# usra-riacs/Nonlocal-Monte-Carlo

Hardware: AMD Instinct MI355X
Metric: spin-updates/s (replicas x spins x sweeps / s), NPT sweep + swap rounds, schedule construction included (higher is better)
Workload: dtype f64 field + 53-bit uniform (the reference's arithmetic, NMC/nmc.py:86-87; on this +-J instance the fp64 field is an exact integer and the fp64 acceptance test an exact integer threshold per field value: bit-identical to the sweep-by-sweep fp64 kernel and the fp64 oracle); 1 GPU; NPT heat-bath sweeps + replica exchange, sparse +-J spin glass (C4 per GPU); spins=10000, edges=30000, replicas_per_gpu=256, replicas_total=256, sweeps_per_round=10, swap_pairs_per_round=77, rng=philox4x32-10, order=one permutation per sweep, plan_chunk_rounds=256

## Files before the change

### nonlocal-monte-carlo_amd/csrc/nlmc.hip

```cpp
#include "../../include/nlmc.h"
#include "nlmc_kernels.h"
#include "nlmc_pt_icm.h"
#include "nlmc_apt.h"
#include "nlmc_lbp.h"
#include "nlmc_nmc.h"
#include "nlmc_probe.h"
#include "nlmc_big.h"
#include "nlmc_host.h"

#include <dlfcn.h>

#include <algorithm>
#include <chrono>
#include <thread>
#include <climits>
#include <cmath>
#include <cstdio>
#include <cstdlib>
#include <cstring>
#include <string>
#include <vector>

namespace {

// ... 443 lines not shown
{
    const int waves = nt / 64;
    if (const char *s = getenv("NLMC_FUSED_GEN0")) { const int v = atoi(s); if (v >= 0 && v < waves) return v; }
    return waves / 2;
}

bool fused_supported(const nlmc_ctx *c, int T)
{
    if (getenv("NLMC_NO_FUSED") || c->big) return false;
    if (c->n < 256 || c->n > NLMC_FZ_SPT * 1024 || c->max_deg > 0x3FFF || T < 3 || T > NLMC_FUSED_TMAX) return false;
    if ((size_t)T * ((size_t)c->n + c->n_long) > ((size_t)1 << 22)) return false;
    if (c->n_pad + 16 > 0x3FFF) return false;
    (void)T;
    const FusedLds L = fused_lds(c->n, c->n_pad, true, false, false);
    if (3 * L.u_bytes / 4 > 0xFFFF) return false;
    return L.total <= (size_t)150 * 1024;
}

bool fused_f64_supported(const nlmc_ctx *c, int T)
{
    if (!c->f64_exact || c->xmax > 4095 || getenv("NLMC_NO_FUSED64")) return false;
    if (!fused_supported(c, T)) return false;
    return fused_lds(c->n, c->n_pad, false, false, fused_addr_format(c), 2 * c->xmax + 1).total <= (size_t)156 * 1024;
}

bool fused_f64_real_supported(const nlmc_ctx *c, int T)
{
    if (!c->f64_real || c->f64_exact || getenv("NLMC_NO_FUSED64")) return false;
    return fused_supported(c, T);
}

bool fused_f64_any(const nlmc_ctx *c, int T) { return fused_f64_supported(c, T) || fused_f64_real_supported(c, T); }

const void *fused_kernel(bool diag, bool flags, bool outs, int fmt, bool f64 = false, bool real = false)
{
    if (f64 && real) {
#define NLMC_KR(D, O) {reinterpret_cast<const void *>(k_sweep_fused<D, false, O, NLMC_FMT_WIDE, true, false, true>), \
                       reinterpret_cast<const void *>(k_sweep_fused<D, false, O, NLMC_FMT_COMPACT, true, false, true>), \
                       reinterpret_cast<const void *>(k_sweep_fused<D, false, O, NLMC_FMT_ADDR, true, false, true>)}
        static const void *const tr[2][2][3] = {{NLMC_KR(false, false), NLMC_KR(false, true)}, {NLMC_KR(true, false), NLMC_KR(true, true)}};
#undef NLMC_KR
        return flags ? nullptr : tr[diag][outs][fmt];
    }
    if (f64) {
#define NLMC_K64(D, O) {reinterpret_cast<const void *>(k_sweep_fused<D, false, O, NLMC_FMT_WIDE, true>), reinterpret_cast<const void *>(k_sweep_fused<D, false, O, NLMC_FMT_COMPACT, true>), \
                        reinterpret_cast<const void *>(k_sweep_fused<D, false, O, NLMC_FMT_ADDR, true>)}
        static const void *const t64[2][2][3] = {{NLMC_K64(false, false), NLMC_K64(false, true)}, {NLMC_K64(true, false), NLMC_K64(true, true)}};
#undef NLMC_K64
        return flags ? nullptr : t64[diag][outs][fmt];
    }
#define NLMC_K(D, F, O) {reinterpret_cast<const void *>(k_sweep_fused<D, F, O, NLMC_FMT_WIDE>), reinterpret_cast<const void *>(k_sweep_fused<D, F, O, NLMC_FMT_COMPACT>), \
                         reinterpret_cast<const void *>(k_sweep_fused<D, F, O, NLMC_FMT_ADDR>)}
    static const void *const table[2][2][2][3] = {{{NLMC_K(false, false, false), NLMC_K(false, false, true)}, {NLMC_K(false, true, false), NLMC_K(false, true, true)}},
                                                  {{NLMC_K(true, false, false), NLMC_K(true, false, true)}, {NLMC_K(true, true, false), NLMC_K(true, true, true)}}};
#undef NLMC_K
    static_assert(NLMC_FMT_WIDE == 0 && NLMC_FMT_COMPACT == 1 && NLMC_FMT_ADDR == 2, "table order");
    return table[diag][flags][outs][fmt];
}

struct SweepOut {
    int record_stride;
    int8_t *out_spins;
    double *out_energy;
    double *out_min_energy;
    int32_t *out_argmin;
    int8_t *out_argmin_state;
// ... 3 lines not shown
              bool outs, bool want_energy, bool want_min, bool want_state, int rec, int t0, int n_total, bool f64 = false,
              const DeferSwap *defer = nullptr, double *sink_override = nullptr)
{
    const nlmc_ctx::FusedPlan &P = c->fz[slot];
    const int R = c->sub_count(), n = c->n, T = P.T;
    const size_t PS = (size_t)P.pstride;
    const bool real = f64 && !c->f64_exact;
    if (real && !P.has_val) return fail(c, NLMC_ERR_STATE, "run_fused: the plan has no fp64 value plane");
    const int kt = (f64 && !real) ? 2 * c->xmax + 1 : 0;
    const bool snap_lds = outs && fused_lds(c->n, c->n_pad, c->has_flags, true, P.fmt == NLMC_FMT_ADDR, kt).total <= (size_t)150 * 1024;
    const FusedLds L = fused_lds(c->n, c->n_pad, c->has_flags, snap_lds, P.fmt == NLMC_FMT_ADDR, kt);
    if (outs && !snap_lds) HIP_TRY(c, c->snap_g.reserve((size_t)R * (3 * (size_t)c->n_pad + 16)));
    const int variant = (outs ? 4 : 0) + (c->has_diag ? 2 : 0) + (c->has_flags ? 1 : 0);
    const void *kfun = fused_kernel(c->has_diag, c->has_flags, outs, P.fmt, f64, real);
    int lds_slot = real ? 84 + ((c->has_diag ? 2 : 0) + (outs ? 1 : 0)) * 3 + P.fmt
                 : f64 ? 48 + ((c->has_diag ? 2 : 0) + (outs ? 1 : 0)) * 3 + P.fmt : 24 + variant * 3 + P.fmt;
    if (defer) {
#define NLMC_KD(D, F64_) {reinterpret_cast<const void *>(k_sweep_fused<D, false, false, NLMC_FMT_WIDE, F64_, true>), reinterpret_cast<const void *>(k_sweep_fused<D, false, false, NLMC_FMT_COMPACT, F64_, true>), \
                          reinterpret_cast<const void *>(k_sweep_fused<D, false, false, NLMC_FMT_ADDR, F64_, true>)}
        static const void *const dtable[2][2][3] = {{NLMC_KD(false, false), NLMC_KD(false, true)}, {NLMC_KD(true, false), NLMC_KD(true, true)}};
#undef NLMC_KD
        kfun = (c->has_flags || outs) ? nullptr : dtable[c->has_diag][f64][P.fmt];
        lds_slot = 72 + ((c->has_diag ? 2 : 0) + (f64 ? 1 : 0)) * 3 + P.fmt;
        if (real) {
#define NLMC_KDR(D) {reinterpret_cast<const void *>(k_sweep_fused<D, false, false, NLMC_FMT_WIDE, true, true, true>), \
                     reinterpret_cast<const void *>(k_sweep_fused<D, false, false, NLMC_FMT_COMPACT, true, true, true>), \
                     reinterpret_cast<const void *>(k_sweep_fused<D, false, false, NLMC_FMT_ADDR, true, true, true>)}
            static const void *const drtable[2][3] = {NLMC_KDR(false), NLMC_KDR(true)};
#undef NLMC_KDR
            kfun = (c->has_flags || outs) ? nullptr : drtable[c->has_diag][P.fmt];
            lds_slot = 96 + (c->has_diag ? 1 : 0) * 3 + P.fmt;
        }
    }
    if (!kfun) return fail(c, NLMC_ERR_STATE, "run_fused: no kernel for this combination (fp64 mode or deferred swap with phase flags / outputs)");
    { int rc = ensure_lds(c, lds_slot, kfun, L.total); if (rc) return rc; }
    const bool timed = c->ev_accumulate && (c->ev_every <= 1 || c->launches_total % c->ev_every == 0);
    hipEvent_t e0 = nullptr, e2 = nullptr;
    if (timed) {
        e0 = next_event(c);
        hipEvent_t e1 = next_event(c);
        e2 = next_event(c);
        if (!e0 || !e1 || !e2) return fail(c, NLMC_ERR_HIP, "hipEventCreate failed");
        tag_triple(c, 1);
        HIP_TRY(c, hipEventRecord(e0, c->cur));
    }
    SweepArgs a{};
    a.g = c->g;
    a.chain_base = c->chain_base;
    a.chain_list = c->sub_list();
    a.spins = c->spins.p;
    a.flags = c->has_flags ? c->flags.p : nullptr;
    a.temp_x = c->temp_x;
    a.lvl_off = P.loff.p + (size_t)w * (NLMC_LCAP + 1);
    a.nlev = P.nlev.p + w;
    a.hi_max = P.himax.p + w;
    a.ell32 = P.ell.p + (size_t)w * PS * NLMC_FZ_W;
    a.head32 = P.head.p + (size_t)w * PS;
    a.fsend = P.send.p + (size_t)w * T;
    a.fz_pstride = P.pstride;
    a.fz_fmt = P.fmt;
    if (w + 1 < P.windows && P.nlev_host[(size_t)w + 1] > 0 && !c->knob_no_warm) {
        a.warm_head = P.head.p + (size_t)(w + 1) * PS;
        a.warm_ell = P.ell.p + (size_t)(w + 1) * PS * NLMC_FZ_W;
        a.fz_npos_next = P.npos_host[(size_t)w + 1];
    }
    a.f_workers = P.workers;
    a.f_gen0 = P.gen0;
    a.f_gen_prio = c->knob_no_prio ? 0 : 1;
#ifdef NLMC_DEBUG_KNOBS
    a.dbg_flags = c->knob_dbg_flags;
#endif
    a.n_sweeps = T;
    a.sweep0 = sweep0;
    a.seed_lo = (uint32_t)seed; a.seed_hi = (uint32_t)(seed >> 32);
    a.tab = tab_dev; a.tab_cs = tab_cs; a.tab_ss = tab_ss;
    a.slot_of_chain = use_slots ? c->slot_of_chain.p : nullptr;
    a.efix = c->efix.p;
    a.energy_sink = sink_override ? sink_override : c->energy_sink;
    if (defer) a.defer = *defer;
    a.escale = c->escale;
    a.eshift = c->escale - c->qs;
    a.qinv = std::ldexp(1.0f, -c->qs);
    a.trace_sweeps = outs ? n_total : T;
    a.t0 = t0;
    a.rec_stride = rec ? rec : 1;
    a.min_stride = c->track_min ? c->track_min_stride : 1;
    a.argmin = c->argmin.p;
    if (outs) {
        a.etrace = want_energy ? c->etrace.p : nullptr;
        a.strace = rec ? c->strace.p : nullptr;
        a.emin = want_min ? c->emin.p : nullptr;
        a.best = (want_min && want_state) ? c->best.p : nullptr;
    }
    a.lds_neg_off = L.neg_off;
    a.lds_flags_off = L.flags_off; a.lds_u_off = L.u_off; a.lds_u_stride = L.u_bytes; a.lds_red_off = L.red_off;
    a.lds_snap_off = L.snap_off;
    a.snap_g = (outs && !snap_lds) ? c->snap_g.p : nullptr;
    a.lds_kt_off = L.kt_off;
    a.f64_xmax = c->xmax;
    a.f64_tie_mask = c->knob_tie_mask;
    a.qinv64 = std::ldexp(1.0, -c->qs);
    a.fz_val = real ? P.val.p + (size_t)w * NLMC_FZ_VAL_WORDS * PS : nullptr;
    a.rng_stride = c->rng_stride; a.rng_base = c->rng_base; a.rng_ladder_len = std::max(1, c->ladder_len);
#ifdef NLMC_STAMPS
    HIP_TRY(c, c->dbg.reserve((size_t)R * 16 * 8 + 96));
    HIP_TRY(c, hipMemsetAsync(c->dbg.p, 0, ((size_t)R * 16 * 8 + 96) * sizeof(long long), c->cur));
    a.dbg = c->dbg.p;
#endif
    const int nt = fused_block(n);
    void *kargs[] = {&a};
    HIP_TRY(c, hipLaunchKernel(kfun, dim3(R), dim3(nt), kargs, L.total, c->cur));
    HIP_TRY(c, hipGetLastError());
    if (timed) { HIP_TRY(c, hipEventRecord(e2, c->cur)); c->launches_timed++; }
    c->launches_sweep++;
    c->launches_total++;
    c->stat_fused_window = w;
    c->stat_fused_slot = slot;
    return NLMC_OK;
}

int read_sweep_outputs(nlmc_ctx *c, const SweepOut &o, int n_sweeps, int rec, int n_rec)
{
    const int R = c->sub_count(), RA = c->n_chains, n = c->n;
    bool need_sync = false;
    std::vector<long long> h_ll;
    if (o.out_energy) {
        h_ll.resize((size_t)R * n_sweeps);
        HIP_TRY(c, hipMemcpyAsync(h_ll.data(), c->etrace.p, sizeof(long long) * h_ll.size(), hipMemcpyDeviceToHost, c->cur));
// ... 2404 lines not shown
```

### nonlocal-monte-carlo_amd/csrc/nlmc_kernels.h

```cpp
#pragma once
#include "nlmc_device.h"

struct EdgeQ { int32_t col; int32_t q; };

struct CsrDev {
    int n, n_pad;
    const int32_t *rowptr;
    const int32_t *col;
    const double *val64;
    const EdgeQ *edge32;
    const double *h64;
    const int32_t *hq;
};

struct LevelizeArgs {
    CsrDev g;
    int n_orders;
    const uint32_t *keys_in;
    uint32_t seed_lo, seed_hi, sweep0;
    int per_chain;
    int n_sweeps;
    int chain_base;
    int level_cap;
    int two_sided;
// ... 1366 lines not shown
#endif
    chain_store(a, x);
}

template <int FMT> struct FusedItem {
    static constexpr int NE = NLMC_FZ_W;
    static constexpr int NP = FMT == NLMC_FMT_WIDE ? NE / 2 : FMT == NLMC_FMT_COMPACT ? NE / 4 : NE / 8;
    nlmc_i2 hd;
    nlmc_i4 pk[NP];
    __device__ __forceinline__ int word(int i) const { const int p = i >> 2, j = i & 3; return j == 0 ? pk[p].x : j == 1 ? pk[p].y : j == 2 ? pk[p].z : pk[p].w; }
    __device__ __forceinline__ unsigned col(int q) const
    {
        if (FMT == NLMC_FMT_WIDE) return (unsigned)word(2 * q);
        if (FMT == NLMC_FMT_COMPACT) return (unsigned)word(q) >> 16;
        return (q & 1) ? (unsigned)word(q >> 1) >> 16 : (unsigned)word(q >> 1) & 0xFFFFu;
    }
    __device__ __forceinline__ int val(int q) const
    {
        if (FMT == NLMC_FMT_WIDE) return word(2 * q + 1);
        return (int)(short)(word(q) & 0xFFFF);
    }
};

__device__ __forceinline__ float4 thresholds4(const u32x4 &r)
{
    float4 v;
    v.x = threshold_spec(r.x);
    v.y = threshold_spec(r.y);
    v.z = threshold_spec(r.z);
    v.w = threshold_spec(r.w);
    return v;
}

struct FusedGenParams { uint32_t gc; int gtid, gnt, nblk, nj, Tn; };
struct FusedWin {
    const int32_t *lvl_off;
    const int32_t *fsend;
    const EdgeQ *ell;
    const int2 *head;
    const int2 *warm_head;
    const EdgeQ *warm_ell;
    int npos_next;
    int nl, hi_max;
    uint32_t sweep0;
    const double *val;
};
struct FusedVals {
    nlmc_i4 v[NLMC_FZ_W / 2];
    nlmc_i2 h;
    __device__ __forceinline__ double val(int q) const
    {
        const nlmc_i4 &w = v[q >> 1];
        return (q & 1) ? __hiloint2double(w.w, w.z) : __hiloint2double(w.y, w.x);
    }
    __device__ __forceinline__ double field() const { return __hiloint2double(h.y, h.x); }
};
template <int CTRL>
__device__ __forceinline__ double quad_move_f64(double v)
{
    const long long b = __double_as_longlong(v);
    const int lo = __builtin_amdgcn_mov_dpp((int)b, CTRL, 0xF, 0xF, true), hi = __builtin_amdgcn_mov_dpp((int)(b >> 32), CTRL, 0xF, 0xF, true);
    return __hiloint2double(hi, lo);
}
#ifdef NLMC_DEBUG_KNOBS
#define NLMC_GEN_DBG_OFF_COND (a.dbg_flags & 1)
#define NLMC_GEN_DBG_PHILOX if (a.dbg_flags & 8) g_r = u32x4{(uint32_t)b * 2654435761u, (uint32_t)b ^ gp.gc, (uint32_t)g_u * 40503u + (uint32_t)b, ~(uint32_t)b}; else
#define NLMC_GEN_DBG_LOGIT if (a.dbg_flags & 16) dst[b] = nlmc_f4{__uint_as_float(g_r.x & 0x3FFFFFFFu), __uint_as_float(g_r.y & 0x3FFFFFFFu), __uint_as_float(g_r.z & 0x3FFFFFFFu), __uint_as_float(g_r.w & 0x3FFFFFFFu)}; else
#else
#define NLMC_GEN_DBG_OFF_COND false
#define NLMC_GEN_DBG_PHILOX
#define NLMC_GEN_DBG_LOGIT
#endif
#define NLMC_GEN_STATE int g_u = 2, g_slot = 2, g_w0 = 0, g_wend = 0, g_wlen = 1, g_acc = 0, g_sidx = 0; u32x4 g_r{0u, 0u, 0u, 0u}; \
    const uint32_t g_seed_lo = a.seed_lo, g_seed_hi = a.seed_hi, g_sweep0 = W.sweep0; const int g_u_off = a.lds_u_off, g_u_stride = a.lds_u_stride; \
    const int32_t *const g_fsend = W.fsend;
#define NLMC_GEN_NSTEP (g_f64 ? 2 : 3)
#define NLMC_GEN_ARM(a, gp)                                                                                             \
    {                                                                                                                   \
        typedef const int32_t __attribute__((address_space(4))) *const_i32_;                                            \
        g_sidx = 0; g_acc = 0;                                                                                          \
        if (g_u < gp.Tn) {                                                                                              \
            const const_i32_ send_ = (const_i32_)(uintptr_t)g_fsend;                                                    \
            g_w0 = g_u >= 3 ? __builtin_amdgcn_readfirstlane(send_[g_u - 3]) : -1;                                      \
            g_wend = __builtin_amdgcn_readfirstlane(send_[g_u - 2]);                                                    \
            g_wlen = max(1, g_wend - g_w0);                 \
        } else g_w0 = 0x7FFFFFFF;                                                                                       \
    }
#define NLMC_GEN_STEP(a, gp)                                                                                            \
    {                                                                                                                   \
        const int call_ = g_sidx / NLMC_GEN_NSTEP, ph_ = g_sidx - call_ * NLMC_GEN_NSTEP;                               \
        const int b = gp.gtid + call_ * gp.gnt;                                                                         \
        if (ph_ == 0) {                                                                                                 \
            NLMC_GEN_DBG_PHILOX                                                                                         \
            g_r = philox4x32_rounds(u32x4{(uint32_t)b, g_sweep0 + (uint32_t)g_u, gp.gc, NLMC_TAG_UNIFORM}, g_seed_lo, g_seed_hi, 0, 5); \
        } else if (g_f64) {                                                                                             \
            typedef nlmc_i4 __attribute__((address_space(3))) *lds_i4_;                                                 \
            g_r = philox4x32_rounds(g_r, g_seed_lo, g_seed_hi, 5, 5);                                                   \
            if (b < gp.nblk) ((lds_i4_)(uintptr_t)(unsigned)(g_u_off + g_slot * g_u_stride))[b] = nlmc_i4{(int)(g_r.x >> 5), (int)(g_r.y >> 5), (int)(g_r.z >> 5), (int)(g_r.w >> 5)}; \
        } else if (ph_ == 1) {                                                                                          \
            NLMC_GEN_DBG_PHILOX                                                                                         \
            g_r = philox4x32_rounds(g_r, g_seed_lo, g_seed_hi, 5, 5);                                                   \
        } else if (b < gp.nblk) {                                                                                       \
            typedef nlmc_f4 __attribute__((address_space(3))) *lds_f4_;             \
            const lds_f4_ dst = (lds_f4_)(uintptr_t)(unsigned)(g_u_off + g_slot * g_u_stride);                  \
            NLMC_GEN_DBG_LOGIT                                                                                          \
            { const float4 t4 = thresholds4(g_r); dst[b] = nlmc_f4{t4.x, t4.y, t4.z, t4.w}; }                           \
        }                                                                                                               \
        ++g_sidx;                                                                                                       \
    }
#define NLMC_GEN(a, gp, l)                                                                                              \
    if (!(NLMC_GEN_DBG_OFF_COND) && (l) > g_w0) {                                                                       \
        g_acc += NLMC_GEN_NSTEP * gp.nj;                                                                                \
        while (g_acc >= g_wlen) { g_acc -= g_wlen; if (g_sidx < NLMC_GEN_NSTEP * gp.nj) NLMC_GEN_STEP(a, gp) }          \
        if (__builtin_expect((l) == g_wend, 0)) {                                                                       \
            while (g_sidx < NLMC_GEN_NSTEP * gp.nj) NLMC_GEN_STEP(a, gp)                                                \
            ++g_u; g_slot = g_slot == 2 ? 0 : g_slot + 1; NLMC_GEN_ARM(a, gp)                                           \
        }                                                                                                               \
    }

template <bool DIAG, bool FLAGS, bool PAIR, bool GEN, int FMT, bool OUT = false, bool F64 = false, bool R64 = false>
__device__ __forceinline__ void fused_levels(const SweepArgs &a, const FusedWin &W, unsigned char *lds_raw, int wv, int lane, int nl, float cq0,
                                             float cq1, long long &e_loc, const FusedGenParams gp, double cb64 = 0.0)
{
    constexpr bool g_f64 = F64;
    static_assert(!(F64 && FLAGS), "fused fp64 windows: plain chains only (a scaled row's field is not an exact integer)");
    static_assert(!R64 || F64, "the real-valued fp64 variant rides on the fp64 uniform tables");
    NLMC_GEN_STATE
    NLMC_GEN_ARM(a, gp)
    typedef const int32_t __attribute__((address_space(4))) *const_i32o;
    typedef const double __attribute__((address_space(4))) *const_f64o;
    const int o_npad = a.g.n_pad, o_b = blockIdx.x, o_c = a.chain_list ? a.chain_list[o_b] : o_b, o_tid = wv * 64 + lane;
    int o_t = 0, o_end = 0;
    unsigned o_lo = 0u;
    long long e_new = 0, E_run = 0, E_min = 0;
    int a_min = 0;
    float cqo0 = cq0, cqo1 = cq1, cqn0 = cq0, cqn1 = cq1;
    const int o_row = a.slot_of_chain ? a.slot_of_chain[a.chain_base + o_c] : o_c;
    int8_t *const snapg = (OUT && a.snap_g) ? a.snap_g + (size_t)o_b * (3 * (size_t)o_npad + 16) : nullptr;
#define NLMC_OCQ(t, j) ((float)((const_f64o)(uintptr_t)a.tab)[(size_t)o_row * a.tab_cs + (size_t)min((t), a.n_sweeps - 1) * a.tab_ss + (j)] * a.qinv)
    if (OUT) {
        o_end = ((const_i32o)(uintptr_t)W.fsend)[0];
        E_run = uniform64(a.efix[o_c]);
        E_min = a.emin ? uniform64(a.emin[o_c]) : 0x7FFFFFFFFFFFFFFFll;
        a_min = a.emin ? __builtin_amdgcn_readfirstlane(a.argmin[o_c]) : 0;
        cqn0 = NLMC_OCQ(1, 0); cqn1 = NLMC_OCQ(1, 1);
    }
    typedef FusedItem<FMT> Item;
    unsigned v_u_off = (unsigned)a.lds_u_off, v_neg_off = (unsigned)a.lds_neg_off;
    int v_eshift = a.eshift;
    asm volatile("" : "+v"(v_u_off), "+v"(v_neg_off), "+v"(v_eshift));
    unsigned v_kt0 = (unsigned)(a.lds_kt_off + 4 * a.f64_xmax), v_tie = a.f64_tie_mask;
    if (F64) asm volatile("" : "+v"(v_kt0), "+v"(v_tie));
    const double v_esc = __longlong_as_double((long long)(1023 + a.escale) << 52);
    const bool r_all_exact = a.f64_tie_mask == 0u;
    typedef const unsigned __attribute__((address_space(3))) *lds_u32;
    constexpr int NP = Item::NP, NE = Item::NE;
    const int plane_bytes = a.fz_pstride * 16;
    const __amdgpu_buffer_rsrc_t r_ell = __builtin_amdgcn_make_buffer_rsrc(const_cast<EdgeQ *>(W.ell), 0, (NLMC_FZ_W / 2) * plane_bytes, 0x00020000);
    const __amdgpu_buffer_rsrc_t r_head = __builtin_amdgcn_make_buffer_rsrc(const_cast<int2 *>(W.head), 0, a.fz_pstride * 8, 0x00020000);
    const __amdgpu_buffer_rsrc_t r_val = __builtin_amdgcn_make_buffer_rsrc(const_cast<double *>(W.val), 0, R64 ? (NLMC_FZ_W / 2) * plane_bytes : 0, 0x00020000);
    const __amdgpu_buffer_rsrc_t r_hval = __builtin_amdgcn_make_buffer_rsrc(const_cast<double *>(W.val) + (R64 ? (size_t)NLMC_FZ_W * a.fz_pstride : 0), 0,
                                                                            R64 ? a.fz_pstride * 8 : 0, 0x00020000);
    typedef const int32_t __attribute__((address_space(4))) *const_i32;
    const const_i32 loffp = (const_i32)(uintptr_t)W.lvl_off;
    auto lo = [&](int i) __attribute__((always_inline)) { return loffp[min(i, nl)]; };
    const int lane16 = lane * 16, oob = 0x7FF00000;
    typedef const int8_t __attribute__((address_space(3))) *lds_i8;
    typedef int8_t __attribute__((address_space(3))) *lds_i8w;
    typedef const uint8_t __attribute__((address_space(3))) *lds_u8;
    typedef const float __attribute__((address_space(3))) *lds_f32;

    auto issue = [&](Item &it, int c, bool has) __attribute__((always_inline)) {
#ifdef NLMC_DEBUG_KNOBS
        if (a.dbg_flags & 32) return;
#endif
        const int v16 = has ? lane16 : oob;
        if constexpr (R64 && FMT == NLMC_FMT_WIDE) {
            it.hd.x = (int)__builtin_amdgcn_raw_buffer_load_b32(r_head, v16 >> 1, c * 512, 0);
            it.hd.y = 0;
#pragma unroll
            for (int q = 0; q < NP; ++q) {
                it.pk[q].x = (int)__builtin_amdgcn_raw_buffer_load_b32(r_ell, v16, c * 1024 + q * plane_bytes, 0);
                it.pk[q].z = (int)__builtin_amdgcn_raw_buffer_load_b32(r_ell, v16, c * 1024 + q * plane_bytes + 8, 0);
                it.pk[q].y = it.pk[q].w = 0;
            }
// ... 79 lines not shown
                    int t_ = tw_ >= 3u * np_ ? 3 : tw_ >= 2u * np_ ? 2 : tw_ >= np_ ? 1 : 0;
                    while (t_ + 3 < a.n_sweeps && lv > ((const_i32s)(uintptr_t)W.fsend)[t_]) t_ += 3;
                    const u32x4 r_ = philox4x32_10(ka >> 2, W.sweep0 + (uint32_t)t_, gp.gc, NLMC_TAG_UNIFORM_LO, a.seed_lo, a.seed_hi);
                    const unsigned lw_ = (ka & 2u) ? ((ka & 1u) ? r_.w : r_.z) : ((ka & 1u) ? r_.y : r_.x);
                    const double u = uniform53_spec(hw << 5, lw_);
                    up = __fma_rn(u, E, u) < 1.0;
                }
            }
            const int sn = up ? 1 : -1, ds = sn - so;
            const long long d = (ds != 0 && !(PAIR && second)) ? fixed_delta_slow(x_true, ds, v_esc) : 0ll;
            *(lds_i8w)(uintptr_t)ka = (int8_t)sn;
            if (FMT == NLMC_FMT_ADDR) *(lds_i8w)(uintptr_t)(ka + v_neg_off) = (int8_t)-sn;
            if (OUT) {
                const unsigned tw = (unsigned)hx >> 16;
                const bool is_old = tw - o_lo < (unsigned)o_npad;
                e_loc += is_old ? d : 0ll;
                e_new += is_old ? 0ll : d;
                if (snapg) snapg[tw] = (int8_t)sn;
                else *(lds_i8w)(uintptr_t)(tw + (unsigned)a.lds_snap_off) = (int8_t)sn;
            } else {
                e_loc += d;
            }
            return;
        }
#ifdef NLMC_DEBUG_KNOBS
        if (a.dbg_flags & 2) { asm volatile("" :: "v"(it.hd.x), "v"(it.pk[0].x), "v"(it.pk[Item::NP - 1].x)); return; }
#endif
        const int hx = it.hd.x;
#ifdef NLMC_DEBUG_KNOBS
        const unsigned ka = (a.dbg_flags & 1024) ? (unsigned)((lane & 31) * 4 + (lane >> 5)) : (unsigned)hx & 0x3FFFu;
        const float wk = *(lds_f32)(uintptr_t)(((a.dbg_flags & 1024) ? (unsigned)(lane * 4) : (((unsigned)hx >> 16) << 2)) + (unsigned)a.lds_u_off);
#else
        const unsigned ka = (unsigned)hx & 0x3FFFu;
        const float wk = *(lds_f32)(uintptr_t)((((unsigned)hx >> 16) << 2) + v_u_off);
#endif
        int so = (int)*(lds_i8)(uintptr_t)ka;
        unsigned f = 0u;
        if (FLAGS) f = (unsigned)*(lds_u8)(uintptr_t)(ka + (unsigned)a.lds_flags_off);
        int sj[NE];
#ifdef NLMC_DEBUG_KNOBS
        if (a.dbg_flags & 512) {
#pragma unroll
            for (int q = 0; q < NE; ++q) sj[q] = (int)*(lds_i8)(uintptr_t)(unsigned)((lane & 31) * 4 + q * 132 + (lane >> 5));
        } else
#endif
        {
#pragma unroll
            for (int q = 0; q < NE; ++q) sj[q] = (int)*(lds_i8)(uintptr_t)it.col(q);
        }
        asm volatile("" : "+v"(so));
        int X0 = it.hd.y, X1 = 0, Xd = 0;
#pragma unroll
        for (int q = 0; q < NE; q += 2) {
            if (FMT == NLMC_FMT_ADDR) {
                X0 += sj[q];
                X1 += sj[q + 1];
            } else {
                X0 += __mul24(it.val(q), sj[q]);
                X1 += __mul24(it.val(q + 1), sj[q + 1]);
            }
        }
        if (DIAG) {
#pragma unroll
            for (int q = 0; q < NE; ++q) {
                if (FMT == NLMC_FMT_ADDR) Xd += (it.col(q) == ka || it.col(q) == ka + v_neg_off) ? sj[q] : 0;
                else Xd += (it.col(q) == ka) ? __mul24(it.val(q), sj[q]) : 0;
            }
        }
        int X = X0 + X1;
        bool second = false;
        if (PAIR) {
            if (__builtin_amdgcn_ballot_w64((hx & 0x4000) != 0) != 0ull) {
                if (hx & 0x4000) {
                    const int rs = a.g.rowptr[ka], re = a.g.rowptr[ka + 1];
#pragma clang loop vectorize(disable) unroll(disable)
                    for (int e = rs + 2 * NLMC_FZ_W; e < re; ++e) {
                        const EdgeQ t = a.g.edge32[e];
                        const int pr = __mul24(t.q, (int)*(lds_i8)(uintptr_t)(unsigned)t.col);
                        X += pr;
                        if (DIAG && (unsigned)t.col == ka) Xd += pr;
                    }
                }
            }
            const bool pair = (hx & 0x8000) != 0;
            const int Xp = __builtin_amdgcn_mov_dpp(X, 0xB1, 0xF, 0xF, true);
            X += pair ? Xp : 0;
            if (DIAG) { const int Xdp = __builtin_amdgcn_mov_dpp(Xd, 0xB1, 0xF, 0xF, true); Xd += pair ? Xdp : 0; }
            second = pair && (lane & 1);
        }
        bool up64 = false;
        if (F64 && !R64) {
            const unsigned hk = __float_as_uint(wk);
            const unsigned kaddr = ((unsigned)X << 2) + v_kt0;
#ifdef NLMC_DEBUG_KNOBS
            const unsigned kh = (a.dbg_flags & 16384) ? (unsigned)(X * 3000000 + 0x4000000) : *(lds_u32)(uintptr_t)kaddr;
#else
            const unsigned kh = *(lds_u32)(uintptr_t)kaddr;
#endif
            up64 = hk < kh;
            const bool tie = ((hk ^ kh) & v_tie) == 0u;
            if (__builtin_expect(__builtin_amdgcn_ballot_w64(tie) != 0ull, 0)) {
                if (tie) {
                    typedef const int32_t __attribute__((address_space(4))) *const_i32s;
                    const unsigned tw_ = (unsigned)hx >> 16, np_ = (unsigned)a.g.n_pad;
                    int t_ = tw_ >= 3u * np_ ? 3 : tw_ >= 2u * np_ ? 2 : tw_ >= np_ ? 1 : 0;
                    while (t_ + 3 < a.n_sweeps && lv > ((const_i32s)(uintptr_t)W.fsend)[t_]) t_ += 3;
                    const u32x4 r_ = philox4x32_10(ka >> 2, W.sweep0 + (uint32_t)t_, gp.gc, NLMC_TAG_UNIFORM_LO, a.seed_lo, a.seed_hi);
                    const unsigned lw_ = (ka & 2u) ? ((ka & 1u) ? r_.w : r_.z) : ((ka & 1u) ? r_.y : r_.x);
                    const unsigned lo_ = lw_ >> 6;
                    const unsigned kl = *(lds_u32)(uintptr_t)(kaddr + 4u * (unsigned)(2 * a.f64_xmax + 1));
                    up64 = hk < kh || (hk == kh && lo_ < kl);
                }
            }
        }
        if (!OUT) {
            const float z = ((FLAGS && f == 1u) ? cq1 : cq0) * (float)X;
            int sn = F64 ? (up64 ? 1 : -1) : (z < wk) ? 1 : -1;
            if (FLAGS) sn = (f >= 2u) ? so : sn;
            const int cv = (PAIR && second) ? 0 : (so - sn) << v_eshift;
            e_loc += (long long)(DIAG ? X - Xd : X) * (long long)cv;
            *(lds_i8w)(uintptr_t)ka = (int8_t)sn;
            if (FMT == NLMC_FMT_ADDR) *(lds_i8w)(uintptr_t)(ka + v_neg_off) = (int8_t)-sn;
        } else {
            const unsigned tw = (unsigned)hx >> 16;
// ... 100 lines not shown
        if (a.energy_sink) a.energy_sink[o_c] = (double)E_run * __longlong_as_double((long long)(1023 - a.escale) << 52);
        if (a.emin) { a.emin[o_c] = E_min; a.argmin[o_c] = a_min; }
    }
}

template <bool FLAGS>
__device__ __forceinline__ void fused_state_load(const SweepArgs &a, unsigned char *lds_raw, int c)
{
    const int n_pad = a.g.n_pad, tid = threadIdx.x, nt = blockDim.x;
    long long *red = reinterpret_cast<long long *>(lds_raw + a.lds_red_off);
    {
        const int4 *src = reinterpret_cast<const int4 *>(a.spins + (size_t)c * n_pad);
        int4 *dst = reinterpret_cast<int4 *>(lds_raw);
        for (int i = tid; i < n_pad / 16; i += nt) dst[i] = src[i];
        if (tid < 4) reinterpret_cast<int *>(lds_raw + n_pad)[tid] = tid < 2 ? 0x01010101 : 0;
        if (a.lds_neg_off) {
            int4 *ndst = reinterpret_cast<int4 *>(lds_raw + a.lds_neg_off);
            for (int i = tid; i < n_pad / 16; i += nt) {
                const int4 v = src[i];
                ndst[i] = make_int4(v.x ^ (int)0xFEFEFEFE, v.y ^ (int)0xFEFEFEFE, v.z ^ (int)0xFEFEFEFE, v.w ^ (int)0xFEFEFEFE);
            }
            if (tid < 4) reinterpret_cast<int *>(lds_raw + a.lds_neg_off + n_pad)[tid] = (int)0xFFFFFFFF;
        }
        if (FLAGS) {
            const int4 *fsrc = reinterpret_cast<const int4 *>(a.flags + (size_t)c * n_pad);
            int4 *fdst = reinterpret_cast<int4 *>(lds_raw + a.lds_flags_off);
            for (int i = tid; i < n_pad / 16; i += nt) fdst[i] = fsrc[i];
            if (tid < 4) reinterpret_cast<int *>(lds_raw + a.lds_flags_off + n_pad)[tid] = 0;
        }
        if (tid < 4) red[tid] = 0;
    }
}

template <bool DIAG, bool FLAGS, bool OUT, int FMT, bool F64, bool R64 = false>
__device__ __forceinline__ void fused_window(const SweepArgs &a, const FusedWin &W, unsigned char *lds_raw, int row, uint32_t gc, long long &e_loc)
{
    constexpr bool g_f64 = F64;
    const int n = a.g.n, tid = threadIdx.x, nt = blockDim.x;
    const int wv = __builtin_amdgcn_readfirstlane(tid >> 6), lane = tid & 63;
    float *ur = reinterpret_cast<float *>(lds_raw + a.lds_u_off);
    const int Tn = a.n_sweeps;
#ifdef NLMC_DEBUG_KNOBS
    const int nl = (a.dbg_flags & 128) ? 0 : W.nl;
#else
    const int nl = W.nl;
#endif
    const float cq0 = (float)a.tab[(size_t)row * a.tab_cs] * a.qinv, cq1 = (float)a.tab[(size_t)row * a.tab_cs + 1] * a.qinv;
#ifdef NLMC_DEBUG_KNOBS
    for (int t = 0; t < ((a.dbg_flags & 1) ? 3 : min(2, Tn)) NLMC_DBG_NOPROLOGUE; ++t) {
#else
    for (int t = 0; t < min(2, Tn) NLMC_DBG_NOPROLOGUE; ++t) {
#endif
        float *tab_t = reinterpret_cast<float *>(reinterpret_cast<unsigned char *>(ur) + (size_t)t * a.lds_u_stride);
        if (F64) fill_uniform_words(reinterpret_cast<unsigned *>(tab_t), n, W.sweep0 + (uint32_t)t, gc, a.seed_lo, a.seed_hi, tid, nt);
        else fill_uniforms(tab_t, n, W.sweep0 + (uint32_t)t, gc, a.seed_lo, a.seed_hi, tid, nt);
    }
    const double cb64 = R64 ? a.tab[(size_t)row * a.tab_cs] : 0.0;
    if (F64 && !R64) {
        const int ne = 2 * a.f64_xmax + 1;
        unsigned *kt = reinterpret_cast<unsigned *>(lds_raw + a.lds_kt_off);
        const double cb = a.tab[(size_t)row * a.tab_cs];
        for (int i = nt - 1 - tid; i < ne; i += nt) {
            const double xf = (double)(i - a.f64_xmax) * a.qinv64;
            const unsigned long long K = accept_count_spec(cb * xf);
            kt[i] = (unsigned)(K >> 26);
            kt[ne + i] = (unsigned)(K & 0x3FFFFFFull);
        }
    }
    __syncthreads();

    const int g0 = a.f_gen0 * 64, nblk = (n + 3) / 4, gnt = nt - g0;
    const int gwave0 = __builtin_amdgcn_readfirstlane((tid - g0) & ~63);
    const FusedGenParams gp{gc, tid - g0, gnt, nblk, max(0, (nblk - gwave0 + gnt - 1) / gnt), Tn};
    const bool is_gen = tid >= g0;
    if (is_gen && a.f_gen_prio) __builtin_amdgcn_s_setprio(2);
    if (wv < a.f_workers) {
        const bool role_long = wv < W.hi_max;
        const int variant = (role_long ? 2 : 0) + (is_gen ? 1 : 0);
#define NLMC_FL(P, G) fused_levels<DIAG, FLAGS, P, G, FMT, OUT, F64, R64>(a, W, lds_raw, wv, lane, nl, cq0, cq1, e_loc, gp, cb64)
        switch (variant) { case 0: NLMC_FL(false, false); break; case 1: NLMC_FL(false, true); break;
                           case 2: NLMC_FL(true, false); break; default: NLMC_FL(true, true); break; }
#undef NLMC_FL
    } else {
        NLMC_GEN_STATE
        NLMC_GEN_ARM(a, gp)
        const int hid = tid - a.f_workers * 64, hcnt = nt - a.f_workers * 64;
        const unsigned warm_lines = W.warm_head ? (unsigned)(((size_t)W.npos_next * 8 + 127) / 128) : 0u;
        const unsigned warm_lines_p = W.warm_head ? (unsigned)(((size_t)a.fz_pstride * 16 + 127) / 128) : 0u;
        const unsigned warm_used_p = W.warm_head ? (unsigned)(((size_t)W.npos_next * 16 + 127) / 128) : 0u;
        const unsigned warm_total = warm_lines + (FMT == NLMC_FMT_ADDR ? 1u : FMT == NLMC_FMT_COMPACT ? 2u : 4u) * warm_used_p;
        unsigned warm_at = (unsigned)blockIdx.x * (unsigned)hcnt + (unsigned)hid;
        const unsigned warm_step = gridDim.x * (unsigned)hcnt;
        unsigned wv0 = 0u, wv1 = 0u, wv2 = 0u, wv3 = 0u;
        auto warm_addr = [&]() __attribute__((always_inline)) -> const unsigned * {
            const char *p = reinterpret_cast<const char *>(W.lvl_off);
            if (warm_at < warm_lines) p = reinterpret_cast<const char *>(W.warm_head) + (size_t)warm_at * 128;
            else if (warm_at < warm_total) {
                const unsigned r = warm_at - warm_lines, q = r / warm_used_p, i = r - q * warm_used_p;
                p = reinterpret_cast<const char *>(W.warm_ell) + ((size_t)q * warm_lines_p + i) * 128;
            }
            warm_at = warm_at < warm_total ? warm_at + warm_step : warm_at;
            return reinterpret_cast<const unsigned *>(p);
        };
#define NLMC_WARM(reg) { asm volatile("" :: "v"(reg) : "memory"); reg = *warm_addr(); }
#ifdef NLMC_STAMPS
        long long sw0, sw1, sw2, st_work = 0, st_bar = 0;
#endif
        for (int l = 0; l < nl; l += 4) {
            NLMC_FW0
            NLMC_WARM(wv0)
            if (is_gen) NLMC_GEN(a, gp, l)
            NLMC_FW1
// ... 61 lines not shown
            partner = __hip_atomic_load(&chain_of_slot[(size_t)g * L + ps], __ATOMIC_RELAXED, __HIP_MEMORY_SCOPE_AGENT);
            Ep = __hip_atomic_load(&e_all[partner], __ATOMIC_RELAXED, __HIP_MEMORY_SCOPE_AGENT);
        } else {
            partner = chain_of_slot[(size_t)g * L + ps];
            Ep = e_all[partner];
        }
        const double Ea = slot == i ? Ed : Ep, Eb = slot == i ? Ep : Ed;
        const double dE = Eb - Ea, dB = beta[i + 1] - beta[i];
        const u32x4 rr = philox4x32_10((uint32_t)fp, round, (uint32_t)g, NLMC_TAG_SWAP, seed_lo, seed_hi);
        const double u = uniform_from(rr, 0.0);
        const double z = (dB * dE) * 1.4426950408889634;
        const bool acc = u < exp2_spec(z);
        if (lane == 0) {
            if (slot == i && log_pairs) {
                const size_t at = (size_t)g * n_pairs + fp;
                log_pairs[2 * at] = i; log_pairs[2 * at + 1] = i + 1;
                log_acc[at] = acc ? 1 : 0;
            }
            if (acc) {
                if (ATOMIC) {
                    __hip_atomic_store(&slot_of_chain[gc], ps, __ATOMIC_RELAXED, __HIP_MEMORY_SCOPE_AGENT);
                    __hip_atomic_store(&chain_of_slot[(size_t)g * L + ps], (int)gc, __ATOMIC_RELAXED, __HIP_MEMORY_SCOPE_AGENT);
                } else {
                    slot_of_chain[gc] = ps;
                    chain_of_slot[(size_t)g * L + ps] = (int)gc;
                }
            }
        }
        if (acc) out = ps;
    }
    return out;
}

template <bool DIAG, bool FLAGS, bool OUT, int FMT, bool F64 = false, bool DEFER = false, bool R64 = false>
__global__ __launch_bounds__(1024) void k_sweep_fused(SweepArgs a)
{
    extern __shared__ __align__(16) unsigned char lds_raw[];
    if ((unsigned)reinterpret_cast<size_t>(lds_raw) != 0u) __builtin_trap();
    static_assert(!(DEFER && OUT), "the deferred swap rides on the plain variant");
    const int c = a.chain_list ? a.chain_list[blockIdx.x] : (int)blockIdx.x;
    const uint32_t gc_chain = (uint32_t)(a.chain_base + c);
    int row = a.slot_of_chain ? a.slot_of_chain[gc_chain] : c;
    int new_row = row;
    if (DEFER && a.defer.n_pairs > 0 && threadIdx.x < 64)
        new_row = pt_swap_step_of_chain<false>(row, gc_chain, (int)threadIdx.x, a.defer.ladder_len, a.defer.n_pairs, a.defer.n_ladders, a.defer.round,
                                               a.defer.plan_pairs, a.defer.beta, a.defer.slot_of_chain, a.defer.chain_of_slot,
                                               a.defer.e_prev[gc_chain], a.defer.e_prev, a.defer.log_pairs, a.defer.log_acc, a.seed_lo, a.seed_hi);
#ifdef NLMC_STAMPS
    const long long st_begin = (long long)__builtin_readcyclecounter();
#endif
    const FusedWin W{a.lvl_off, a.fsend, a.ell32, a.head32, a.warm_head, a.warm_ell, a.fz_npos_next, a.nlev[0], a.hi_max[0], a.sweep0, a.fz_val};
    fused_state_load<FLAGS>(a, lds_raw, c);
    if (DEFER) {
        volatile int *sh = reinterpret_cast<volatile int *>(lds_raw + a.lds_red_off);
        __syncthreads();
        if (threadIdx.x == 0) sh[0] = new_row;
        __syncthreads();
        row = sh[0];
        __syncthreads();
        if (threadIdx.x == 0) sh[0] = 0;
    }
    const uint32_t gc = (a.rng_stride && a.slot_of_chain) ? (uint32_t)((c / a.rng_ladder_len) * a.rng_stride + a.rng_base + row) : gc_chain;
    long long e_loc = 0;
    fused_window<DIAG, FLAGS, OUT, FMT, F64, R64>(a, W, lds_raw, row, gc, e_loc);
    fused_state_store<OUT>(a, lds_raw, c, e_loc);
#ifdef NLMC_STAMPS
    if (a.dbg && (threadIdx.x & 63) == 0) a.dbg[((size_t)blockIdx.x * 16 + (threadIdx.x >> 6)) * 8 + 7] = (long long)__builtin_readcyclecounter() - st_begin;
#endif
}

struct RoundsArgs {
    int n_rounds, n_windows_avail;
    const int32_t *loff, *nlev, *himax, *send, *npos;
    const int2 *head;
    const EdgeQ *ell;
    int ladder_len, n_pairs, n_ladders;
    uint32_t round0;
    const int32_t *plan_pairs;
    const double *beta;
    int32_t *slot_of_chain, *chain_of_slot;
    double *ebuf;
    int32_t *log_pairs;
    uint8_t *log_acc;
    unsigned *bar;
    int32_t *status;
    long long timeout_ticks;
};

__device__ __forceinline__ bool grid_arrive_and_wait(unsigned *bar, unsigned target, int32_t *status, long long t_end, volatile int *flag)
{
    if (threadIdx.x == 0) {
        asm volatile("s_waitcnt vmcnt(0)" ::: "memory");
        __hip_atomic_fetch_add(bar, 1u, __ATOMIC_RELAXED, __HIP_MEMORY_SCOPE_AGENT);
        int good = 1;
        while (__hip_atomic_load(bar, __ATOMIC_RELAXED, __HIP_MEMORY_SCOPE_AGENT) < target) {
            if (__hip_atomic_load(status, __ATOMIC_RELAXED, __HIP_MEMORY_SCOPE_AGENT) == 3 || (long long)wall_clock64() > t_end) {
                __hip_atomic_store(status, 3, __ATOMIC_RELAXED, __HIP_MEMORY_SCOPE_AGENT);
// ... 170 lines not shown
```

Baseline: 224.8 billion spin-updates/s.

## Precompute per-spin decision-threshold bytes in generator waves for fp64 sweeps

For the integer-field fp64 mode, generator waves now turn each 53-bit uniform into a one-byte rank threshold over the field values. They use a float log estimate checked against the key table, and fall back to an exact binary search with the low Philox word when there is a tie. The sweep workers then decide a flip with one byte compare instead of loading the uniform word and indexing the key table. This moves work onto the generator waves (an extra Philox step plus the log and rank checks) and shrinks LDS per slot to one byte per spin. It is enabled only for the address format with xmax<=126.

```diff
diff --git a/nonlocal-monte-carlo_amd/csrc/nlmc.hip b/nonlocal-monte-carlo_amd/csrc/nlmc.hip
--- a/nonlocal-monte-carlo_amd/csrc/nlmc.hip
+++ b/nonlocal-monte-carlo_amd/csrc/nlmc.hip
@@ -499,6 +499,11 @@
 
 bool fused_f64_any(const nlmc_ctx *c, int T) { return fused_f64_supported(c, T) || fused_f64_real_supported(c, T); }
 
+bool fused_rank_bytes(const nlmc_ctx *c, int fmt, bool outs)
+{
+    return fmt == NLMC_FMT_ADDR && !outs && !c->has_flags && c->f64_exact && c->xmax <= 126 && !getenv("NLMC_NO_LDS_STREAM");
+}
+
 const void *fused_kernel(bool diag, bool flags, bool outs, int fmt, bool f64 = false, bool real = false)
 {
     if (f64 && real) {
@@ -568,6 +573,15 @@
             lds_slot = 96 + (c->has_diag ? 1 : 0) * 3 + P.fmt;
         }
     }
+    const bool rb = f64 && !real && fused_rank_bytes(c, P.fmt, outs);
+    if (rb) {
+#define NLMC_KB(D) {reinterpret_cast<const void *>(k_sweep_fused<D, false, false, NLMC_FMT_ADDR, true, false, false, true>), \
+                    reinterpret_cast<const void *>(k_sweep_fused<D, false, false, NLMC_FMT_ADDR, true, true, false, true>)}
+        static const void *const btable[2][2] = {NLMC_KB(false), NLMC_KB(true)};
+#undef NLMC_KB
+        kfun = btable[c->has_diag][defer ? 1 : 0];
+        lds_slot = 102 + (c->has_diag ? 2 : 0) + (defer ? 1 : 0);
+    }
     if (!kfun) return fail(c, NLMC_ERR_STATE, "run_fused: no kernel for this combination (fp64 mode or deferred swap with phase flags / outputs)");
     { int rc = ensure_lds(c, lds_slot, kfun, L.total); if (rc) return rc; }
     const bool timed = c->ev_accumulate && (c->ev_every <= 1 || c->launches_total % c->ev_every == 0);
@@ -629,7 +643,7 @@
         a.best = (want_min && want_state) ? c->best.p : nullptr;
     }
     a.lds_neg_off = L.neg_off;
-    a.lds_flags_off = L.flags_off; a.lds_u_off = L.u_off; a.lds_u_stride = L.u_bytes; a.lds_red_off = L.red_off;
+    a.lds_flags_off = L.flags_off; a.lds_u_off = L.u_off; a.lds_u_stride = rb ? c->n_pad : L.u_bytes; a.lds_red_off = L.red_off;
     a.lds_snap_off = L.snap_off;
     a.snap_g = (outs && !snap_lds) ? c->snap_g.p : nullptr;
     a.lds_kt_off = L.kt_off;
diff --git a/nonlocal-monte-carlo_amd/csrc/nlmc_kernels.h b/nonlocal-monte-carlo_amd/csrc/nlmc_kernels.h
--- a/nonlocal-monte-carlo_amd/csrc/nlmc_kernels.h
+++ b/nonlocal-monte-carlo_amd/csrc/nlmc_kernels.h
@@ -1422,7 +1422,75 @@
     return v;
 }
 
-struct FusedGenParams { uint32_t gc; int gtid, gnt, nblk, nj, Tn; };
+struct RankTab { unsigned kt; int ne, xmax, flip; unsigned tmask; float tsc; };
+struct FusedGenParams { uint32_t gc; int gtid, gnt, nblk, nj, Tn; RankTab rt; };
+__device__ __forceinline__ unsigned rank_khi(const RankTab &R, int j)
+{
+    typedef const unsigned __attribute__((address_space(3))) *lds_u32_;
+    return *(lds_u32_)(uintptr_t)(R.kt + 4u * (unsigned)(R.flip ? j : R.ne - 1 - j));
+}
+__device__ __forceinline__ unsigned long long rank_k53(const RankTab &R, int j)
+{
+    typedef const unsigned __attribute__((address_space(3))) *lds_u32_;
+    const unsigned a = R.kt + 4u * (unsigned)(R.flip ? j : R.ne - 1 - j);
+    return ((unsigned long long)*(lds_u32_)(uintptr_t)a << 26) | *(lds_u32_)(uintptr_t)(a + 4u * (unsigned)R.ne);
+}
+__device__ __attribute__((noinline)) unsigned rank_bytes4_exact(unsigned kt, int ne, int xmax, int flip, unsigned tmask, unsigned r0, unsigned r1,
+                                                                unsigned r2, unsigned r3, uint32_t b, uint32_t tt, uint32_t gc, uint32_t k0, uint32_t k1)
+{
+    const RankTab R{kt, ne, xmax, flip, tmask, 0.0f};
+    const unsigned hk[4] = {r0 >> 5, r1 >> 5, r2 >> 5, r3 >> 5};
+    int c[4];
+    bool tie[4];
+    for (int q = 0; q < 4; ++q) {
+        const unsigned hm = hk[q] & tmask;
+        int lo = 0, hi = ne;
+        while (lo < hi) { const int mid = (lo + hi) >> 1; if ((rank_khi(R, mid) & tmask) >= hm) lo = mid + 1; else hi = mid; }
+        c[q] = lo;
+        tie[q] = lo > 0 && (rank_khi(R, lo - 1) & tmask) == hm;
+    }
+    if (tie[0] || tie[1] || tie[2] || tie[3]) {
+        const u32x4 l = philox4x32_10(b, tt, gc, NLMC_TAG_UNIFORM_LO, k0, k1);
+        const unsigned lw[4] = {l.x, l.y, l.z, l.w};
+        for (int q = 0; q < 4; ++q) {
+            if (tie[q]) {
+                const unsigned long long u53 = ((unsigned long long)hk[q] << 26) | (lw[q] >> 6);
+                int lo = 0, hi = ne;
+                while (lo < hi) { const int mid = (lo + hi) >> 1; if (rank_k53(R, mid) > u53) lo = mid + 1; else hi = mid; }
+                c[q] = lo;
+            }
+        }
+    }
+    unsigned out = 0u;
+    for (int q = 0; q < 4; ++q) out |= ((unsigned)(xmax + 1 - c[q] - flip) & 0xFFu) << (8 * q);
+    return out;
+}
+__device__ __forceinline__ unsigned rank_bytes4(const RankTab &R, const u32x4 &r, uint32_t b, uint32_t tt, uint32_t gc, uint32_t k0, uint32_t k1)
+{
+    const unsigned hk[4] = {r.x >> 5, r.y >> 5, r.z >> 5, r.w >> 5};
+    int c[4];
+    unsigned ka[4], kc[4];
+#pragma unroll
+    for (int q = 0; q < 4; ++q) {
+        const float u = ((float)hk[q] + 0.5f) * 0x1p-27f;
+        const float t = __log2f(__frcp_rn(u) - 1.0f) * R.tsc;
+        float g = R.flip ? (float)R.xmax + ceilf(t) : (float)R.xmax - floorf(t);
+        g = fminf(fmaxf(g, 0.0f), (float)R.ne);
+        c[q] = (int)g;
+        ka[q] = rank_khi(R, max(c[q] - 1, 0));
+        kc[q] = rank_khi(R, min(c[q], R.ne - 1));
+    }
+    bool ok = true;
+    unsigned out = 0u;
+#pragma unroll
+    for (int q = 0; q < 4; ++q) {
+        const unsigned hm = hk[q] & R.tmask;
+        ok = ok && (c[q] == 0 || (ka[q] & R.tmask) > hm) && (c[q] == R.ne || (kc[q] & R.tmask) < hm);
+        out |= ((unsigned)(R.xmax + 1 - c[q] - R.flip) & 0xFFu) << (8 * q);
+    }
+    if (__builtin_expect(!ok, 0)) out = rank_bytes4_exact(R.kt, R.ne, R.xmax, R.flip, R.tmask, r.x, r.y, r.z, r.w, b, tt, gc, k0, k1);
+    return out;
+}
 struct FusedWin {
     const int32_t *lvl_off;
     const int32_t *fsend;
@@ -1464,7 +1532,7 @@
 #define NLMC_GEN_STATE int g_u = 2, g_slot = 2, g_w0 = 0, g_wend = 0, g_wlen = 1, g_acc = 0, g_sidx = 0; u32x4 g_r{0u, 0u, 0u, 0u}; \
     const uint32_t g_seed_lo = a.seed_lo, g_seed_hi = a.seed_hi, g_sweep0 = W.sweep0; const int g_u_off = a.lds_u_off, g_u_stride = a.lds_u_stride; \
     const int32_t *const g_fsend = W.fsend;
-#define NLMC_GEN_NSTEP (g_f64 ? 2 : 3)
+#define NLMC_GEN_NSTEP (g_f64 && !g_rb ? 2 : 3)
 #define NLMC_GEN_ARM(a, gp)                                                                                             \
     {                                                                                                                   \
         typedef const int32_t __attribute__((address_space(4))) *const_i32_;                                            \
@@ -1483,13 +1551,17 @@
         if (ph_ == 0) {                                                                                                 \
             NLMC_GEN_DBG_PHILOX                                                                                         \
             g_r = philox4x32_rounds(u32x4{(uint32_t)b, g_sweep0 + (uint32_t)g_u, gp.gc, NLMC_TAG_UNIFORM}, g_seed_lo, g_seed_hi, 0, 5); \
-        } else if (g_f64) {                                                                                             \
+        } else if (g_f64 && !g_rb) {                                                                                    \
             typedef nlmc_i4 __attribute__((address_space(3))) *lds_i4_;                                                 \
             g_r = philox4x32_rounds(g_r, g_seed_lo, g_seed_hi, 5, 5);                                                   \
             if (b < gp.nblk) ((lds_i4_)(uintptr_t)(unsigned)(g_u_off + g_slot * g_u_stride))[b] = nlmc_i4{(int)(g_r.x >> 5), (int)(g_r.y >> 5), (int)(g_r.z >> 5), (int)(g_r.w >> 5)}; \
         } else if (ph_ == 1) {                                                                                          \
             NLMC_GEN_DBG_PHILOX                                                                                         \
             g_r = philox4x32_rounds(g_r, g_seed_lo, g_seed_hi, 5, 5);                                                   \
+        } else if (g_rb) {                                                                                              \
+            typedef unsigned __attribute__((address_space(3))) *lds_u32w_;                                              \
+            if (b < gp.nblk) ((lds_u32w_)(uintptr_t)(unsigned)(g_u_off + g_slot * g_u_stride))[b] =                     \
+                rank_bytes4(gp.rt, g_r, (uint32_t)b, g_sweep0 + (uint32_t)g_u, gp.gc, g_seed_lo, g_seed_hi);            \
         } else if (b < gp.nblk) {                                                                                       \
             typedef nlmc_f4 __attribute__((address_space(3))) *lds_f4_;             \
             const lds_f4_ dst = (lds_f4_)(uintptr_t)(unsigned)(g_u_off + g_slot * g_u_stride);                  \
@@ -1508,13 +1580,14 @@
         }                                                                                                               \
     }
 
-template <bool DIAG, bool FLAGS, bool PAIR, bool GEN, int FMT, bool OUT = false, bool F64 = false, bool R64 = false>
+template <bool DIAG, bool FLAGS, bool PAIR, bool GEN, int FMT, bool OUT = false, bool F64 = false, bool R64 = false, bool RB = false>
 __device__ __forceinline__ void fused_levels(const SweepArgs &a, const FusedWin &W, unsigned char *lds_raw, int wv, int lane, int nl, float cq0,
                                              float cq1, long long &e_loc, const FusedGenParams gp, double cb64 = 0.0)
 {
-    constexpr bool g_f64 = F64;
+    constexpr bool g_f64 = F64, g_rb = RB;
     static_assert(!(F64 && FLAGS), "fused fp64 windows: plain chains only (a scaled row's field is not an exact integer)");
     static_assert(!R64 || F64, "the real-valued fp64 variant rides on the fp64 uniform tables");
+    static_assert(!RB || (F64 && !R64 && !OUT), "decision bytes: the integer-field fp64 mode, plain variant");
     NLMC_GEN_STATE
     NLMC_GEN_ARM(a, gp)
     typedef const int32_t __attribute__((address_space(4))) *const_i32o;
@@ -1540,7 +1613,8 @@
     int v_eshift = a.eshift;
     asm volatile("" : "+v"(v_u_off), "+v"(v_neg_off), "+v"(v_eshift));
     unsigned v_kt0 = (unsigned)(a.lds_kt_off + 4 * a.f64_xmax), v_tie = a.f64_tie_mask;
-    if (F64) asm volatile("" : "+v"(v_kt0), "+v"(v_tie));
+    if (F64 && !RB) asm volatile("" : "+v"(v_kt0), "+v"(v_tie));
+    const int v_flip = -gp.rt.flip;
     const double v_esc = __longlong_as_double((long long)(1023 + a.escale) << 52);
     const bool r_all_exact = a.f64_tie_mask == 0u;
     typedef const unsigned __attribute__((address_space(3))) *lds_u32;
@@ -1686,9 +1760,10 @@
         const float wk = *(lds_f32)(uintptr_t)(((a.dbg_flags & 1024) ? (unsigned)(lane * 4) : (((unsigned)hx >> 16) << 2)) + (unsigned)a.lds_u_off);
 #else
         const unsigned ka = (unsigned)hx & 0x3FFFu;
-        const float wk = *(lds_f32)(uintptr_t)((((unsigned)hx >> 16) << 2) + v_u_off);
+        const float wk = RB ? 0.0f : *(lds_f32)(uintptr_t)((((unsigned)hx >> 16) << 2) + v_u_off);
 #endif
         int so = (int)*(lds_i8)(uintptr_t)ka;
+        int rk = RB ? (int)*(lds_i8)(uintptr_t)(((unsigned)hx >> 16) + v_u_off) : 0;
         unsigned f = 0u;
         if (FLAGS) f = (unsigned)*(lds_u8)(uintptr_t)(ka + (unsigned)a.lds_flags_off);
         int sj[NE];
@@ -1703,6 +1778,7 @@
             for (int q = 0; q < NE; ++q) sj[q] = (int)*(lds_i8)(uintptr_t)it.col(q);
         }
         asm volatile("" : "+v"(so));
+        if (RB) asm volatile("" : "+v"(rk));
         int X0 = it.hd.y, X1 = 0, Xd = 0;
 #pragma unroll
         for (int q = 0; q < NE; q += 2) {
@@ -1743,7 +1819,9 @@
             second = pair && (lane & 1);
         }
         bool up64 = false;
-        if (F64 && !R64) {
+        if (RB) {
+            up64 = (X ^ v_flip) >= rk;
+        } else if (F64 && !R64) {
             const unsigned hk = __float_as_uint(wk);
             const unsigned kaddr = ((unsigned)X << 2) + v_kt0;
 #ifdef NLMC_DEBUG_KNOBS
@@ -1910,10 +1988,10 @@
     }
 }
 
-template <bool DIAG, bool FLAGS, bool OUT, int FMT, bool F64, bool R64 = false>
+template <bool DIAG, bool FLAGS, bool OUT, int FMT, bool F64, bool R64 = false, bool RB = false>
 __device__ __forceinline__ void fused_window(const SweepArgs &a, const FusedWin &W, unsigned char *lds_raw, int row, uint32_t gc, long long &e_loc)
 {
-    constexpr bool g_f64 = F64;
+    constexpr bool g_f64 = F64, g_rb = RB;
     const int n = a.g.n, tid = threadIdx.x, nt = blockDim.x;
     const int wv = __builtin_amdgcn_readfirstlane(tid >> 6), lane = tid & 63;
     float *ur = reinterpret_cast<float *>(lds_raw + a.lds_u_off);
@@ -1927,7 +2005,7 @@
 #ifdef NLMC_DEBUG_KNOBS
     for (int t = 0; t < ((a.dbg_flags & 1) ? 3 : min(2, Tn)) NLMC_DBG_NOPROLOGUE; ++t) {
 #else
-    for (int t = 0; t < min(2, Tn) NLMC_DBG_NOPROLOGUE; ++t) {
+    for (int t = 0; t < (RB ? 0 : min(2, Tn)) NLMC_DBG_NOPROLOGUE; ++t) {
 #endif
         float *tab_t = reinterpret_cast<float *>(reinterpret_cast<unsigned char *>(ur) + (size_t)t * a.lds_u_stride);
         if (F64) fill_uniform_words(reinterpret_cast<unsigned *>(tab_t), n, W.sweep0 + (uint32_t)t, gc, a.seed_lo, a.seed_hi, tid, nt);
@@ -1945,17 +2023,31 @@
             kt[ne + i] = (unsigned)(K & 0x3FFFFFFull);
         }
     }
+    RankTab rt{};
+    if (RB) {
+        const double cb = a.tab[(size_t)row * a.tab_cs];
+        rt = RankTab{(unsigned)a.lds_kt_off, 2 * a.f64_xmax + 1, a.f64_xmax, cb > 0.0 ? 1 : 0, a.f64_tie_mask, (float)(1.0 / (cb * a.qinv64))};
+        __syncthreads();
+        const int nb = (n + 3) / 4;
+        for (int t = 0; t < min(2, Tn); ++t) {
+            unsigned *tab_t = reinterpret_cast<unsigned *>(lds_raw + a.lds_u_off + (size_t)t * a.lds_u_stride);
+            for (int b = tid; b < nb; b += nt) {
+                const u32x4 r = philox4x32_10((uint32_t)b, W.sweep0 + (uint32_t)t, gc, NLMC_TAG_UNIFORM, a.seed_lo, a.seed_hi);
+                tab_t[b] = rank_bytes4(rt, r, (uint32_t)b, W.sweep0 + (uint32_t)t, gc, a.seed_lo, a.seed_hi);
+            }
+        }
+    }
     __syncthreads();
 
     const int g0 = a.f_gen0 * 64, nblk = (n + 3) / 4, gnt = nt - g0;
     const int gwave0 = __builtin_amdgcn_readfirstlane((tid - g0) & ~63);
-    const FusedGenParams gp{gc, tid - g0, gnt, nblk, max(0, (nblk - gwave0 + gnt - 1) / gnt), Tn};
+    const FusedGenParams gp{gc, tid - g0, gnt, nblk, max(0, (nblk - gwave0 + gnt - 1) / gnt), Tn, rt};
     const bool is_gen = tid >= g0;
     if (is_gen && a.f_gen_prio) __builtin_amdgcn_s_setprio(2);
     if (wv < a.f_workers) {
         const bool role_long = wv < W.hi_max;
         const int variant = (role_long ? 2 : 0) + (is_gen ? 1 : 0);
-#define NLMC_FL(P, G) fused_levels<DIAG, FLAGS, P, G, FMT, OUT, F64, R64>(a, W, lds_raw, wv, lane, nl, cq0, cq1, e_loc, gp, cb64)
+#define NLMC_FL(P, G) fused_levels<DIAG, FLAGS, P, G, FMT, OUT, F64, R64, RB>(a, W, lds_raw, wv, lane, nl, cq0, cq1, e_loc, gp, cb64)
         switch (variant) { case 0: NLMC_FL(false, false); break; case 1: NLMC_FL(false, true); break;
                            case 2: NLMC_FL(true, false); break; default: NLMC_FL(true, true); break; }
 #undef NLMC_FL
@@ -2083,7 +2175,7 @@
     return out;
 }
 
-template <bool DIAG, bool FLAGS, bool OUT, int FMT, bool F64 = false, bool DEFER = false, bool R64 = false>
+template <bool DIAG, bool FLAGS, bool OUT, int FMT, bool F64 = false, bool DEFER = false, bool R64 = false, bool RB = false>
 __global__ __launch_bounds__(1024) void k_sweep_fused(SweepArgs a)
 {
     extern __shared__ __align__(16) unsigned char lds_raw[];
@@ -2113,7 +2205,7 @@
     }
     const uint32_t gc = (a.rng_stride && a.slot_of_chain) ? (uint32_t)((c / a.rng_ladder_len) * a.rng_stride + a.rng_base + row) : gc_chain;
     long long e_loc = 0;
-    fused_window<DIAG, FLAGS, OUT, FMT, F64, R64>(a, W, lds_raw, row, gc, e_loc);
+    fused_window<DIAG, FLAGS, OUT, FMT, F64, R64, RB>(a, W, lds_raw, row, gc, e_loc);
     fused_state_store<OUT>(a, lds_raw, c, e_loc);
 #ifdef NLMC_STAMPS
     if (a.dbg && (threadIdx.x & 63) == 0) a.dbg[((size_t)blockIdx.x * 16 + (threadIdx.x >> 6)) * 8 + 7] = (long long)__builtin_readcyclecounter() - st_begin;
```

Result: slower. 177.5 billion spin-updates/s (median of 2 runs) (-21.0%).
